# andrewcharlesjones/spatial-alignment

Hardware: AMD Instinct MI355X
Metric: training steps/sec (ELBO fwd+bwd), 2-view N=10k M=200, 1/2/4/8 GPU (higher is better)
Workload: dtype f32 (fp64 warp layer, covariance whitening and M x M factorisations)

## Files before the change

spatial_alignment_amd/csrc/longk64.hip:

```cpp
#include <stdlib.h>
#include <string.h>

#include "internal.hpp"

namespace gpsa {

typedef double lk_f64x4 __attribute__((ext_vector_type(4)));
typedef double lk_f64x2 __attribute__((ext_vector_type(2)));
typedef float lk_f32x2 __attribute__((ext_vector_type(2)));
typedef __attribute__((address_space(3))) void* lk_lds_ptr;

constexpr int LK_WAVES = 8;
constexpr int LK_MAXP = 48;

struct LongKArgs {
  const double* G[LK_MAXP];
  const double* B[LK_MAXP];
  const void* d[LK_MAXP];
  double* part;
  int M, nprob, nsplit, sym;
  long long K, ld, gper;
};

__device__ __forceinline__ void lk_set_m0(unsigned lds_base) {
  asm volatile("s_mov_b32 m0, %0\n\ts_nop 0" ::"s"(lds_base) : "memory");
}
template <int IMM>
__device__ __forceinline__ void lk_glds16(const void* gsrc_minus_imm) {
  asm volatile("global_load_lds_dwordx4 %0, off offset:%1" ::"v"(gsrc_minus_imm), "n"(IMM) : "memory");
}
template <int IMM>
__device__ __forceinline__ void lk_glds4(const void* gsrc_minus_imm) {
  asm volatile("global_load_lds_dword %0, off offset:%1" ::"v"(gsrc_minus_imm), "n"(IMM) : "memory");
}

template <int MB, bool HASG, int DT>
__global__ void __launch_bounds__(512) longk64_kernel(LongKArgs a) {
  static_assert(HASG || DT != 0, "a left operand");
  constexpr int MP = MB * 16;
  constexpr int NOPD = HASG ? 2 : 1;
  constexpr int NPIECE = MB * NOPD * 2;
  constexpr int NPW = (NPIECE + LK_WAVES - 1) / LK_WAVES;
  static_assert(NPW <= 8, "two groups of four pieces per wave (an immediate offset reaches 4 KiB)");
  constexpr int DAREA = DT == 2 ? 1024 : 256;
  constexpr int STAGE_B = NPW * LK_WAVES * 1024 + (DT ? LK_WAVES * DAREA : 0);
  constexpr int NT_MAX = (MB * MB + LK_WAVES - 1) / LK_WAVES;
  constexpr int NT_SYM = (MB * (MB + 1) / 2 + LK_WAVES - 1) / LK_WAVES;
  extern __shared__ __attribute__((aligned(16))) char lk_smem[];

  const int tid = threadIdx.x, lane = tid & 63;
  const int w = __builtin_amdgcn_readfirstlane(tid >> 6);
  const int li = lane & 15, kq = lane >> 4;
  const int p = blockIdx.y, sp = blockIdx.x;
  const int M = a.M;
  const long long K = a.K, ld = a.ld;
  const double* __restrict__ Bp = a.B[p];
  const double* __restrict__ Gp = HASG ? a.G[p] : nullptr;
  const long long ng = (K + 15) >> 4;
  const long long g_lo = (long long)sp * a.gper;
  long long g_hi = g_lo + a.gper;
  if (g_hi > ng) g_hi = ng;
  const unsigned lds0 = (unsigned)(unsigned long long)(lk_lds_ptr)(&lk_smem[0]);

  const int T = a.sym ? MB * (MB + 1) / 2 : MB * MB;
  const int t_lo = w * T / LK_WAVES, t_hi = (w + 1) * T / LK_WAVES;
  const int cnt = t_hi - t_lo;
  int i0 = 0, j0 = 0;
  if (a.sym) {
    while ((i0 + 1) * (i0 + 2) / 2 <= t_lo) ++i0;
    j0 = t_lo - i0 * (i0 + 1) / 2;
  } else {
    i0 = t_lo / MB;
    j0 = t_lo - i0 * MB;
  }
  if (cnt == 0) i0 = j0 = 0;

  const double* rp[NPW];
  int koff[NPW];
#pragma unroll
  for (int u = 0; u < NPW; ++u) {
    int q = w + LK_WAVES * u;
    q = q < NPIECE ? q : NPIECE - 1;
    const int h = q & 1, ot = q >> 1;
    const bool isg = HASG && ot >= MB;
    const int t = isg ? ot - MB : ot;
    int row = t * 16 + li;
    row = row < M ? row : M - 1;
    rp[u] = (isg ? Gp : Bp) + (long long)row * ld;
    koff[u] = 8 * h + 2 * kq;
  }

  auto issue = [&](long long g, int s) {
    const long long kb = g << 4;
#pragma unroll
    for (int u = 0; u < NPW; ++u) {
      if ((u & 3) == 0)
        lk_set_m0(__builtin_amdgcn_readfirstlane(lds0 + (unsigned)(s * STAGE_B + (w * NPW + u) * 1024)));
      long long k = kb + koff[u];
      k = k < K - 2 ? k : K - 2;
      const char* src = reinterpret_cast<const char*>(rp[u] + k);
      switch (u & 3) {
        case 0: lk_glds16<0>(src); break;
        case 1: lk_glds16<1024>(src - 1024); break;
        case 2: lk_glds16<2048>(src - 2048); break;
        default: lk_glds16<3072>(src - 3072); break;
      }
    }
    if (DT != 0) {
      lk_set_m0(__builtin_amdgcn_readfirstlane(lds0 + (unsigned)(s * STAGE_B + NPW * LK_WAVES * 1024 + w * DAREA)));
      if (DT == 1) {
        long long k = kb + (lane & 15);
        k = k < K ? k : K - 1;
        lk_glds4<0>(reinterpret_cast<const float*>(a.d[p]) + k);
      } else {
        long long k = kb + 2 * (lane & 7);
        k = k < K - 1 ? k : K - 2;
        lk_glds16<0>(reinterpret_cast<const double*>(a.d[p]) + k);
      }
    }
  };

  lk_f64x4 acc[NT_MAX];
#pragma unroll
  for (int t = 0; t < NT_MAX; ++t) acc[t] = (lk_f64x4){0.0, 0.0, 0.0, 0.0};

  if (g_lo < g_hi) {
    issue(g_lo, 0);
    int s = 0;
    for (long long g = g_lo; g < g_hi; ++g) {
      asm volatile("s_waitcnt vmcnt(0)" ::: "memory");
      __syncthreads();
      if (g + 1 < g_hi) issue(g + 1, s ^ 1);
      const char* slot = lk_smem + s * STAGE_B;
      const char* dslot = slot + NPW * LK_WAVES * 1024 + w * DAREA;
      const long long k_a = (g << 4) + 2 * kq;
      double dv[2][2] = {{1.0, 1.0}, {1.0, 1.0}};
      bool ok[2][2];
#pragma unroll
      for (int h = 0; h < 2; ++h) {
        ok[h][0] = k_a + 8 * h < K;
        ok[h][1] = k_a + 8 * h + 1 < K;
        if (DT == 1) {
          const lk_f32x2 x = *reinterpret_cast<const lk_f32x2*>(dslot + 4 * (8 * h + 2 * kq));
          dv[h][0] = (double)x.x;
          dv[h][1] = (double)x.y;
        } else if (DT == 2) {
          const lk_f64x2 x = *reinterpret_cast<const lk_f64x2*>(dslot + 8 * (8 * h + 2 * kq));
          dv[h][0] = x.x;
          dv[h][1] = x.y;
        }
      }
#define LK_FRAG(O, TL, H)                                                                              \
  (*reinterpret_cast<const lk_f64x2*>(slot + ((((((O) * MB + (TL)) * 2 + (H)) & 7) * NPW +             \
                                                 ((((O) * MB + (TL)) * 2 + (H)) >> 3)) << 10) + lane * 16))
      int i = i0, j = j0, cur = -1;
      double af[2][2] = {{0.0, 0.0}, {0.0, 0.0}};
      lk_f64x2 bn0 = LK_FRAG(0, j, 0), bn1 = LK_FRAG(0, j, 1);
#pragma unroll
      for (int t = 0; t < NT_MAX; ++t) {
        if (t >= NT_SYM && a.sym) break;
        if (i != cur) {
          cur = i;
#pragma unroll
          for (int h = 0; h < 2; ++h) {
            const lk_f64x2 bi = LK_FRAG(0, i, h);
            double x0, x1;
            if (HASG) {
              const lk_f64x2 gi = LK_FRAG(1, i, h);
              x0 = DT ? fma(dv[h][0], bi.x, gi.x) : gi.x;
              x1 = DT ? fma(dv[h][1], bi.y, gi.y) : gi.y;
            } else {
              x0 = dv[h][0] * bi.x;
              x1 = dv[h][1] * bi.y;
            }
            af[h][0] = ok[h][0] ? x0 : 0.0;
            af[h][1] = ok[h][1] ? x1 : 0.0;
          }
        }
        const lk_f64x2 b0 = bn0, b1 = bn1;
        if (t + 1 < cnt) {
          ++j;
          if (a.sym ? j > i : j == MB) {
            ++i;
            j = 0;
          }
        }
        if (t + 1 < NT_MAX) {
          bn0 = LK_FRAG(0, j, 0);
          bn1 = LK_FRAG(0, j, 1);
        }
        acc[t] = __builtin_amdgcn_mfma_f64_16x16x4f64(af[0][0], b0.x, acc[t], 0, 0, 0);
        acc[t] = __builtin_amdgcn_mfma_f64_16x16x4f64(af[0][1], b0.y, acc[t], 0, 0, 0);
        acc[t] = __builtin_amdgcn_mfma_f64_16x16x4f64(af[1][0], b1.x, acc[t], 0, 0, 0);
        acc[t] = __builtin_amdgcn_mfma_f64_16x16x4f64(af[1][1], b1.y, acc[t], 0, 0, 0);
      }
#undef LK_FRAG
      s ^= 1;
    }
  }
  double* __restrict__ out = a.part + ((long long)p * a.nsplit + sp) * MP * MP;
  int i = i0, j = j0;
#pragma unroll
  for (int t = 0; t < NT_MAX; ++t) {
    if (t < cnt) {
#pragma unroll
      for (int r = 0; r < 4; ++r) out[(long long)(i * 16 + kq + 4 * r) * MP + j * 16 + li] = acc[t][r];
      ++j;
      if (a.sym ? j > i : j == MB) {
        ++i;
        j = 0;
      }
    }
  }
}

struct LongKOut {
  double* out[LK_MAXP];
  double alpha[LK_MAXP], beta[LK_MAXP];
};

__global__ void __launch_bounds__(256)
longk64_reduce_kernel(const double* __restrict__ part, int M, int MP, int nsplit, int sym, LongKOut o) {
  __shared__ double red[4][64];
  const int lane = threadIdx.x & 63, grp = threadIdx.x >> 6;
  const int p = blockIdx.y;
  const long long e = blockIdx.x * 64LL + lane;
  const int r = (int)(e / M), c = (int)(e % M);
  const bool ok = e < (long long)M * M && !(sym && c > r);
  const long long mm = (long long)MP * MP;
  const double* q = part + (long long)p * nsplit * mm + (long long)r * MP + c;
  double a0 = 0.0, a1 = 0.0, a2 = 0.0, a3 = 0.0;
  if (ok) {
    int s = grp;
    for (; s + 12 < nsplit; s += 16) {
      a0 += q[s * mm];
      a1 += q[(s + 4) * mm];
      a2 += q[(s + 8) * mm];
      a3 += q[(s + 12) * mm];
    }
    for (; s < nsplit; s += 4) a0 += q[s * mm];
  }
  red[grp][lane] = (a0 + a1) + (a2 + a3);
  __syncthreads();
  if (grp == 0 && ok) {
    const double sum = (red[0][lane] + red[1][lane]) + (red[2][lane] + red[3][lane]);
    const double al = o.alpha[p], be = o.beta[p];
    double* dst = o.out[p] + (long long)r * M + c;
    *dst = (be == 0.0) ? al * sum : al * sum + be * (*dst);
    if (sym && c < r) {
      double* dm = o.out[p] + (long long)c * M + r;
      *dm = (be == 0.0) ? al * sum : al * sum + be * (*dm);
    }
  }
}

static inline int longk_mb_for(int M) {
  const int mb = (M + 15) / 16;
  if (mb <= 2) return 2;
  if (mb <= 4) return 4;
  if (mb <= 7) return 7;
  if (mb <= 13) return 13;
  if (mb <= 16) return 16;
  return 0;
}

static inline int longk_nsplit(long long K, int nprob) {
  const long long ng = (K + 15) / 16;
  long long s = (long long)num_cus() / (nprob > 0 ? nprob : 1);
  if (s > ng / 4) s = ng / 4;
  return (int)(s < 1 ? 1 : s);
}

template <int MB, bool HASG, int DT>
static int longk64_launch_mb(const LongKArgs& a, hipStream_t st) {
  constexpr int NPIECE = MB * (HASG ? 2 : 1) * 2, NPW = (NPIECE + LK_WAVES - 1) / LK_WAVES;
  constexpr int lds = 2 * (NPW * LK_WAVES * 1024 + (DT ? LK_WAVES * (DT == 2 ? 1024 : 256) : 0));
  static per_device_flag attr_flag;
  bool& attr_set = attr_flag.here();
  if (!attr_set) {
    if (hipFuncSetAttribute(reinterpret_cast<const void*>(&longk64_kernel<MB, HASG, DT>),
                            hipFuncAttributeMaxDynamicSharedMemorySize, lds) != hipSuccess)
      return GPSA_EUNSUPPORTED;
    attr_set = true;
  }
  dim3 grid((unsigned)a.nsplit, (unsigned)a.nprob);
  longk64_kernel<MB, HASG, DT><<<grid, 512, lds, st>>>(a);
  GPSA_LAUNCH_CHECK();
  return 0;
}

template <bool HASG, int DT>
static int longk64_launch(int MB, const LongKArgs& a, hipStream_t st) {
  switch (MB) {
    case 2: return longk64_launch_mb<2, HASG, DT>(a, st);
    case 4: return longk64_launch_mb<4, HASG, DT>(a, st);
    case 7: return longk64_launch_mb<7, HASG, DT>(a, st);
    case 13: return longk64_launch_mb<13, HASG, DT>(a, st);
    case 16: return longk64_launch_mb<16, HASG, DT>(a, st);
    default: return GPSA_EUNSUPPORTED;
  }
}

}

extern "C" {

long long gpsa_longk_f64_workspace(int M, long long K, int nprob) {
  using namespace gpsa;
  const int MB = longk_mb_for(M);
  if (MB == 0 || nprob < 1 || nprob > LK_MAXP || K < 512 || (K & 1)) return 0;
  const int ns = longk_nsplit(K, nprob);
  if ((long long)ns * nprob < 48) return 0;
  return (long long)nprob * ns * MB * 16 * MB * 16 * 8;
}

int gpsa_longk_f64(int nprob, const double* const* G, const double* const* B, const void* const* d, int d_dtype,
                   int M, long long K, long long ld, int sym, const double* alpha, const double* beta,
                   double* const* out, void* workspace, long long workspace_bytes, void* stream) {
  using namespace gpsa;
  if (nprob < 1 || nprob > LK_MAXP || !B || !out || !alpha || !beta || M < 1 || K < 2 || ld < K) return GPSA_EINVAL;
  if (d != nullptr && d_dtype != GPSA_F32 && d_dtype != GPSA_F64) return GPSA_EINVAL;
  if (G == nullptr && d == nullptr) return GPSA_EINVAL;
  const long long need = gpsa_longk_f64_workspace(M, K, nprob);
  if (need == 0 || (ld & 1)) return GPSA_EUNSUPPORTED;
  if (workspace_bytes < need) return GPSA_EWORKSPACE;
  const int MB = longk_mb_for(M);
  LongKArgs a;
  LongKOut o;
  memset(&a, 0, sizeof(a));
  memset(&o, 0, sizeof(o));
  for (int p = 0; p < nprob; ++p) {
    a.B[p] = B[p];
    a.G[p] = G ? G[p] : nullptr;
    a.d[p] = d ? d[p] : nullptr;
    if (!B[p] || !out[p] || (G && !G[p]) || (d && !d[p])) return GPSA_EINVAL;
    if ((reinterpret_cast<uintptr_t>(B[p]) & 15) || (G && (reinterpret_cast<uintptr_t>(G[p]) & 15)) ||
        (d && d_dtype == GPSA_F64 && (reinterpret_cast<uintptr_t>(d[p]) & 15)))
      return GPSA_EUNSUPPORTED;
    o.out[p] = out[p];
    o.alpha[p] = alpha[p];
    o.beta[p] = beta[p];
  }
  a.part = reinterpret_cast<double*>(workspace);
  a.M = M;
  a.nprob = nprob;
  a.nsplit = longk_nsplit(K, nprob);
  a.sym = sym ? 1 : 0;
  a.K = K;
  a.ld = ld;
  a.gper = cdiv(cdiv(K, 16), a.nsplit);
  hipStream_t st = as_stream(stream);
  int rc;
  if (G && d && d_dtype == GPSA_F32) rc = longk64_launch<true, 1>(MB, a, st);
  else if (G && d) rc = longk64_launch<true, 2>(MB, a, st);
  else if (G) rc = longk64_launch<true, 0>(MB, a, st);
  else if (d_dtype == GPSA_F32) rc = longk64_launch<false, 1>(MB, a, st);
  else rc = longk64_launch<false, 2>(MB, a, st);
  if (rc) return rc;
  dim3 rg((unsigned)cdiv((long long)M * M, 64), (unsigned)nprob);
  longk64_reduce_kernel<<<rg, 256, 0, st>>>(a.part, M, MB * 16, a.nsplit, a.sym, o);
  GPSA_LAUNCH_CHECK();
  return 0;
}

}
```

Baseline: 149.1.

## Specialise long-K f64 MFMA kernel per wave with compile-time tile plans

Builds a constexpr per-wave tile schedule (row/column indices and when to prefetch the next A row) and instantiates a separate code path per wave index and per symmetric/non-symmetric mode. Full K-groups run without the ragged-edge masking, and only the final partial group takes the masked path. The intent is to remove runtime index arithmetic, dead accumulator registers and masking selects from the inner MFMA loop, and to schedule LDS fragment loads ahead of the MFMAs. In exchange, code size grows through eight wave-specialised bodies per template combination, and more kernel variants must be compiled.

```diff
diff --git a/spatial_alignment_amd/csrc/longk64.hip b/spatial_alignment_amd/csrc/longk64.hip
--- a/spatial_alignment_amd/csrc/longk64.hip
+++ b/spatial_alignment_amd/csrc/longk64.hip
@@ -34,9 +34,148 @@
   asm volatile("global_load_lds_dword %0, off offset:%1" ::"v"(gsrc_minus_imm), "n"(IMM) : "memory");
 }
 
-template <int MB, bool HASG, int DT>
-__global__ void __launch_bounds__(512) longk64_kernel(LongKArgs a) {
-  static_assert(HASG || DT != 0, "a left operand");
+template <int MB, bool SYM>
+struct LongKPlan {
+  static constexpr int T = SYM ? MB * (MB + 1) / 2 : MB * MB;
+  static constexpr int NT = (T + LK_WAVES - 1) / LK_WAVES;
+  int cnt[LK_WAVES];
+  int ti[LK_WAVES][NT], tj[LK_WAVES][NT], req[LK_WAVES][NT];
+  bool ok;
+  constexpr LongKPlan() : cnt{}, ti{}, tj{}, req{}, ok(true) {
+    int t = 0;
+    for (int i = 0; i < MB; ++i)
+      for (int j = 0; j < (SYM ? i + 1 : MB); ++j, ++t)
+        for (int w = 0; w < LK_WAVES; ++w)
+          if (t >= w * T / LK_WAVES && t < (w + 1) * T / LK_WAVES) {
+            ti[w][cnt[w]] = i;
+            tj[w][cnt[w]] = j;
+            ++cnt[w];
+          }
+    for (int w = 0; w < LK_WAVES; ++w) {
+      int prev = -1;
+      for (int s = 0; s < NT; ++s) req[w][s] = -1;
+      for (int c = 0; c + 1 < cnt[w]; ++c)
+        if (ti[w][c + 1] != ti[w][c]) {
+          const int at = c - 1 > prev + 1 ? c - 1 : prev + 1;
+          req[w][at] = ti[w][c + 1];
+          prev = c;
+        }
+    }
+    int owned[MB * MB] = {};
+    int total = 0;
+    for (int w = 0; w < LK_WAVES; ++w) {
+      const int t_lo = w * T / LK_WAVES, t_hi = (w + 1) * T / LK_WAVES;
+      if (cnt[w] != t_hi - t_lo || cnt[w] > NT) ok = false;
+      int i = 0, j = 0;
+      if (SYM) {
+        while ((i + 1) * (i + 2) / 2 <= t_lo) ++i;
+        j = t_lo - i * (i + 1) / 2;
+      } else {
+        i = t_lo / MB;
+        j = t_lo - i * MB;
+      }
+      for (int s = 0; s < cnt[w]; ++s) {
+        if (ti[w][s] != i || tj[w][s] != j) ok = false;
+        ++owned[i * MB + j];
+        ++total;
+        ++j;
+        if (SYM ? j > i : j == MB) {
+          ++i;
+          j = 0;
+        }
+      }
+    }
+    for (int i = 0; i < MB; ++i)
+      for (int j = 0; j < MB; ++j)
+        if (owned[i * MB + j] != ((SYM && j > i) ? 0 : 1)) ok = false;
+    if (total != T) ok = false;
+  }
+};
+
+template <int MB, bool HASG, int DT, bool SYM, int W, bool RAGGED, int NA>
+__device__ __forceinline__ void longk_wave_stage(const char* slot, const char* dslot, int lane, int kq, long long k_a,
+                                                 long long K, lk_f64x4 (&acc)[NA]) {
+  constexpr LongKPlan<MB, SYM> P{};
+  constexpr int N = P.cnt[W];
+  constexpr int NPIECE = MB * (HASG ? 2 : 1) * 2, NPW = (NPIECE + LK_WAVES - 1) / LK_WAVES;
+  if (N == 0) return;
+  const char* fb = slot + lane * 16;
+  auto frag = [&](int o, int tl, int h) {
+    const int q = (o * MB + tl) * 2 + h;
+    return *reinterpret_cast<const lk_f64x2*>(fb + (((q & 7) * NPW + (q >> 3)) << 10));
+  };
+  double dv[2][2] = {{1.0, 1.0}, {1.0, 1.0}};
+  bool ok[2][2] = {{true, true}, {true, true}};
+  lk_f64x2 braw[2], graw[2];
+  double af[2][2];
+  auto fetch_row = [&](int i) {
+#pragma unroll
+    for (int h = 0; h < 2; ++h) {
+      if (DT != 0) braw[h] = frag(0, i, h);
+      if (HASG) graw[h] = frag(1, i, h);
+    }
+  };
+  auto form_row = [&]() {
+#pragma unroll
+    for (int h = 0; h < 2; ++h) {
+      double x0, x1;
+      if (HASG) {
+        x0 = DT ? fma(dv[h][0], braw[h].x, graw[h].x) : graw[h].x;
+        x1 = DT ? fma(dv[h][1], braw[h].y, graw[h].y) : graw[h].y;
+      } else {
+        x0 = dv[h][0] * braw[h].x;
+        x1 = dv[h][1] * braw[h].y;
+      }
+      af[h][0] = RAGGED ? (ok[h][0] ? x0 : 0.0) : x0;
+      af[h][1] = RAGGED ? (ok[h][1] ? x1 : 0.0) : x1;
+    }
+  };
+  fetch_row(P.ti[W][0]);
+  lk_f64x2 bn0 = frag(0, P.tj[W][0], 0), bn1 = frag(0, P.tj[W][0], 1);
+#pragma unroll
+  for (int h = 0; h < 2; ++h) {
+    if (RAGGED) {
+      ok[h][0] = k_a + 8 * h < K;
+      ok[h][1] = k_a + 8 * h + 1 < K;
+    }
+    if (DT == 1) {
+      const lk_f32x2 x = *reinterpret_cast<const lk_f32x2*>(dslot + 4 * (8 * h + 2 * kq));
+      dv[h][0] = (double)x.x;
+      dv[h][1] = (double)x.y;
+    } else if (DT == 2) {
+      const lk_f64x2 x = *reinterpret_cast<const lk_f64x2*>(dslot + 8 * (8 * h + 2 * kq));
+      dv[h][0] = x.x;
+      dv[h][1] = x.y;
+    }
+  }
+  form_row();
+#pragma unroll
+  for (int t = 0; t < N; ++t) {
+    const lk_f64x2 b0 = bn0, b1 = bn1;
+    if (t + 1 < N) {
+      bn0 = frag(0, P.tj[W][t + 1], 0);
+      bn1 = frag(0, P.tj[W][t + 1], 1);
+    }
+    if (P.req[W][t] >= 0) fetch_row(P.req[W][t]);
+    __builtin_amdgcn_sched_barrier(0);
+    acc[t] = __builtin_amdgcn_mfma_f64_16x16x4f64(af[0][0], b0.x, acc[t], 0, 0, 0);
+    acc[t] = __builtin_amdgcn_mfma_f64_16x16x4f64(af[0][1], b0.y, acc[t], 0, 0, 0);
+    acc[t] = __builtin_amdgcn_mfma_f64_16x16x4f64(af[1][0], b1.x, acc[t], 0, 0, 0);
+    acc[t] = __builtin_amdgcn_mfma_f64_16x16x4f64(af[1][1], b1.y, acc[t], 0, 0, 0);
+    if (t + 1 < N && P.ti[W][t + 1] != P.ti[W][t]) {
+      __builtin_amdgcn_sched_barrier(0);
+      form_row();
+    }
+    __builtin_amdgcn_sched_barrier(0);
+  }
+}
+
+template <int MB, bool HASG, int DT, bool SYM, int W>
+__device__ __forceinline__ void longk_wave_run(const LongKArgs& a, char* lk_smem) {
+  constexpr LongKPlan<MB, SYM> P{};
+  static_assert(P.ok, "every tile is owned by one wave, in the runs [w T / 8, (w + 1) T / 8) of the row-major list");
+  constexpr int N = P.cnt[W], NA = N > 0 ? N : 1;
+  constexpr int w = W;
   constexpr int MP = MB * 16;
   constexpr int NOPD = HASG ? 2 : 1;
   constexpr int NPIECE = MB * NOPD * 2;
@@ -44,12 +183,8 @@
   static_assert(NPW <= 8, "two groups of four pieces per wave (an immediate offset reaches 4 KiB)");
   constexpr int DAREA = DT == 2 ? 1024 : 256;
   constexpr int STAGE_B = NPW * LK_WAVES * 1024 + (DT ? LK_WAVES * DAREA : 0);
-  constexpr int NT_MAX = (MB * MB + LK_WAVES - 1) / LK_WAVES;
-  constexpr int NT_SYM = (MB * (MB + 1) / 2 + LK_WAVES - 1) / LK_WAVES;
-  extern __shared__ __attribute__((aligned(16))) char lk_smem[];
-
-  const int tid = threadIdx.x, lane = tid & 63;
-  const int w = __builtin_amdgcn_readfirstlane(tid >> 6);
+
+  const int lane = threadIdx.x & 63;
   const int li = lane & 15, kq = lane >> 4;
   const int p = blockIdx.y, sp = blockIdx.x;
   const int M = a.M;
@@ -61,19 +196,6 @@
   long long g_hi = g_lo + a.gper;
   if (g_hi > ng) g_hi = ng;
   const unsigned lds0 = (unsigned)(unsigned long long)(lk_lds_ptr)(&lk_smem[0]);
-
-  const int T = a.sym ? MB * (MB + 1) / 2 : MB * MB;
-  const int t_lo = w * T / LK_WAVES, t_hi = (w + 1) * T / LK_WAVES;
-  const int cnt = t_hi - t_lo;
-  int i0 = 0, j0 = 0;
-  if (a.sym) {
-    while ((i0 + 1) * (i0 + 2) / 2 <= t_lo) ++i0;
-    j0 = t_lo - i0 * (i0 + 1) / 2;
-  } else {
-    i0 = t_lo / MB;
-    j0 = t_lo - i0 * MB;
-  }
-  if (cnt == 0) i0 = j0 = 0;
 
   const double* rp[NPW];
   int koff[NPW];
@@ -120,97 +242,54 @@
     }
   };
 
-  lk_f64x4 acc[NT_MAX];
-#pragma unroll
-  for (int t = 0; t < NT_MAX; ++t) acc[t] = (lk_f64x4){0.0, 0.0, 0.0, 0.0};
+  lk_f64x4 acc[NA];
+#pragma unroll
+  for (int t = 0; t < NA; ++t) acc[t] = (lk_f64x4){0.0, 0.0, 0.0, 0.0};
 
   if (g_lo < g_hi) {
     issue(g_lo, 0);
     int s = 0;
-    for (long long g = g_lo; g < g_hi; ++g) {
+    const long long g_full = g_hi < (K >> 4) ? g_hi : (K >> 4);
+    long long g = g_lo;
+    for (; g < g_full; ++g) {
       asm volatile("s_waitcnt vmcnt(0)" ::: "memory");
       __syncthreads();
       if (g + 1 < g_hi) issue(g + 1, s ^ 1);
       const char* slot = lk_smem + s * STAGE_B;
-      const char* dslot = slot + NPW * LK_WAVES * 1024 + w * DAREA;
-      const long long k_a = (g << 4) + 2 * kq;
-      double dv[2][2] = {{1.0, 1.0}, {1.0, 1.0}};
-      bool ok[2][2];
-#pragma unroll
-      for (int h = 0; h < 2; ++h) {
-        ok[h][0] = k_a + 8 * h < K;
-        ok[h][1] = k_a + 8 * h + 1 < K;
-        if (DT == 1) {
-          const lk_f32x2 x = *reinterpret_cast<const lk_f32x2*>(dslot + 4 * (8 * h + 2 * kq));
-          dv[h][0] = (double)x.x;
-          dv[h][1] = (double)x.y;
-        } else if (DT == 2) {
-          const lk_f64x2 x = *reinterpret_cast<const lk_f64x2*>(dslot + 8 * (8 * h + 2 * kq));
-          dv[h][0] = x.x;
-          dv[h][1] = x.y;
-        }
-      }
-#define LK_FRAG(O, TL, H)                                                                              \
-  (*reinterpret_cast<const lk_f64x2*>(slot + ((((((O) * MB + (TL)) * 2 + (H)) & 7) * NPW +             \
-                                                 ((((O) * MB + (TL)) * 2 + (H)) >> 3)) << 10) + lane * 16))
-      int i = i0, j = j0, cur = -1;
-      double af[2][2] = {{0.0, 0.0}, {0.0, 0.0}};
-      lk_f64x2 bn0 = LK_FRAG(0, j, 0), bn1 = LK_FRAG(0, j, 1);
-#pragma unroll
-      for (int t = 0; t < NT_MAX; ++t) {
-        if (t >= NT_SYM && a.sym) break;
-        if (i != cur) {
-          cur = i;
-#pragma unroll
-          for (int h = 0; h < 2; ++h) {
-            const lk_f64x2 bi = LK_FRAG(0, i, h);
-            double x0, x1;
-            if (HASG) {
-              const lk_f64x2 gi = LK_FRAG(1, i, h);
-              x0 = DT ? fma(dv[h][0], bi.x, gi.x) : gi.x;
-              x1 = DT ? fma(dv[h][1], bi.y, gi.y) : gi.y;
-            } else {
-              x0 = dv[h][0] * bi.x;
-              x1 = dv[h][1] * bi.y;
-            }
-            af[h][0] = ok[h][0] ? x0 : 0.0;
-            af[h][1] = ok[h][1] ? x1 : 0.0;
-          }
-        }
-        const lk_f64x2 b0 = bn0, b1 = bn1;
-        if (t + 1 < cnt) {
-          ++j;
-          if (a.sym ? j > i : j == MB) {
-            ++i;
-            j = 0;
-          }
-        }
-        if (t + 1 < NT_MAX) {
-          bn0 = LK_FRAG(0, j, 0);
-          bn1 = LK_FRAG(0, j, 1);
-        }
-        acc[t] = __builtin_amdgcn_mfma_f64_16x16x4f64(af[0][0], b0.x, acc[t], 0, 0, 0);
-        acc[t] = __builtin_amdgcn_mfma_f64_16x16x4f64(af[0][1], b0.y, acc[t], 0, 0, 0);
-        acc[t] = __builtin_amdgcn_mfma_f64_16x16x4f64(af[1][0], b1.x, acc[t], 0, 0, 0);
-        acc[t] = __builtin_amdgcn_mfma_f64_16x16x4f64(af[1][1], b1.y, acc[t], 0, 0, 0);
-      }
-#undef LK_FRAG
+      longk_wave_stage<MB, HASG, DT, SYM, W, false, NA>(slot, slot + NPW * LK_WAVES * 1024 + w * DAREA, lane, kq,
+                                                        (g << 4) + 2 * kq, K, acc);
       s ^= 1;
     }
+    if (g < g_hi) {
+      asm volatile("s_waitcnt vmcnt(0)" ::: "memory");
+      __syncthreads();
+      const char* slot = lk_smem + s * STAGE_B;
+      longk_wave_stage<MB, HASG, DT, SYM, W, true, NA>(slot, slot + NPW * LK_WAVES * 1024 + w * DAREA, lane, kq,
+                                                       (g << 4) + 2 * kq, K, acc);
+    }
   }
   double* __restrict__ out = a.part + ((long long)p * a.nsplit + sp) * MP * MP;
-  int i = i0, j = j0;
-#pragma unroll
-  for (int t = 0; t < NT_MAX; ++t) {
-    if (t < cnt) {
-#pragma unroll
-      for (int r = 0; r < 4; ++r) out[(long long)(i * 16 + kq + 4 * r) * MP + j * 16 + li] = acc[t][r];
-      ++j;
-      if (a.sym ? j > i : j == MB) {
-        ++i;
-        j = 0;
-      }
-    }
+#pragma unroll
+  for (int t = 0; t < N; ++t)
+#pragma unroll
+    for (int r = 0; r < 4; ++r)
+      out[(long long)(P.ti[W][t] * 16 + kq + 4 * r) * MP + P.tj[W][t] * 16 + li] = acc[t][r];
+}
+
+template <int MB, bool HASG, int DT, bool SYM>
+__global__ void __launch_bounds__(512) longk64_kernel(LongKArgs a) {
+  static_assert(HASG || DT != 0, "a left operand");
+  extern __shared__ __attribute__((aligned(16))) char lk_smem[];
+  const int w = __builtin_amdgcn_readfirstlane(threadIdx.x >> 6);
+  switch (w) {
+    case 0: longk_wave_run<MB, HASG, DT, SYM, 0>(a, lk_smem); break;
+    case 1: longk_wave_run<MB, HASG, DT, SYM, 1>(a, lk_smem); break;
+    case 2: longk_wave_run<MB, HASG, DT, SYM, 2>(a, lk_smem); break;
+    case 3: longk_wave_run<MB, HASG, DT, SYM, 3>(a, lk_smem); break;
+    case 4: longk_wave_run<MB, HASG, DT, SYM, 4>(a, lk_smem); break;
+    case 5: longk_wave_run<MB, HASG, DT, SYM, 5>(a, lk_smem); break;
+    case 6: longk_wave_run<MB, HASG, DT, SYM, 6>(a, lk_smem); break;
+    default: longk_wave_run<MB, HASG, DT, SYM, 7>(a, lk_smem); break;
   }
 }
 
@@ -271,34 +350,39 @@
   return (int)(s < 1 ? 1 : s);
 }
 
-template <int MB, bool HASG, int DT>
+template <int MB, bool HASG, int DT, bool SYM>
 static int longk64_launch_mb(const LongKArgs& a, hipStream_t st) {
   constexpr int NPIECE = MB * (HASG ? 2 : 1) * 2, NPW = (NPIECE + LK_WAVES - 1) / LK_WAVES;
   constexpr int lds = 2 * (NPW * LK_WAVES * 1024 + (DT ? LK_WAVES * (DT == 2 ? 1024 : 256) : 0));
   static per_device_flag attr_flag;
   bool& attr_set = attr_flag.here();
   if (!attr_set) {
-    if (hipFuncSetAttribute(reinterpret_cast<const void*>(&longk64_kernel<MB, HASG, DT>),
+    if (hipFuncSetAttribute(reinterpret_cast<const void*>(&longk64_kernel<MB, HASG, DT, SYM>),
                             hipFuncAttributeMaxDynamicSharedMemorySize, lds) != hipSuccess)
       return GPSA_EUNSUPPORTED;
     attr_set = true;
   }
   dim3 grid((unsigned)a.nsplit, (unsigned)a.nprob);
-  longk64_kernel<MB, HASG, DT><<<grid, 512, lds, st>>>(a);
+  longk64_kernel<MB, HASG, DT, SYM><<<grid, 512, lds, st>>>(a);
   GPSA_LAUNCH_CHECK();
   return 0;
 }
 
+template <bool HASG, int DT, bool SYM>
+static int longk64_launch_sym(int MB, const LongKArgs& a, hipStream_t st) {
+  switch (MB) {
+    case 2: return longk64_launch_mb<2, HASG, DT, SYM>(a, st);
+    case 4: return longk64_launch_mb<4, HASG, DT, SYM>(a, st);
+    case 7: return longk64_launch_mb<7, HASG, DT, SYM>(a, st);
+    case 13: return longk64_launch_mb<13, HASG, DT, SYM>(a, st);
+    case 16: return longk64_launch_mb<16, HASG, DT, SYM>(a, st);
+    default: return GPSA_EUNSUPPORTED;
+  }
+}
+
 template <bool HASG, int DT>
 static int longk64_launch(int MB, const LongKArgs& a, hipStream_t st) {
-  switch (MB) {
-    case 2: return longk64_launch_mb<2, HASG, DT>(a, st);
-    case 4: return longk64_launch_mb<4, HASG, DT>(a, st);
-    case 7: return longk64_launch_mb<7, HASG, DT>(a, st);
-    case 13: return longk64_launch_mb<13, HASG, DT>(a, st);
-    case 16: return longk64_launch_mb<16, HASG, DT>(a, st);
-    default: return GPSA_EUNSUPPORTED;
-  }
+  return a.sym ? longk64_launch_sym<HASG, DT, true>(MB, a, st) : longk64_launch_sym<HASG, DT, false>(MB, a, st);
 }
 
 }
```

New measurement: 150.1, median of 3. Within noise of the previous version (+0.7%).
